# 2Retr0/GodotOceanWaves

Hardware: AMD Instinct MI355X
Metric: displacement+normal maps/sec, 1024^2 x 4 cascades; achieved HBM GB/s vs peak (higher is better)
Workload: dtype f32; 1 GPU; 1024^2 x 4 cascades per GPU, steady-state tick (modulate + 2-D IFFT + unpack/foam), delta=1/50 s, SURVEY 8d cascade table; map_size=1024, cascades_per_gpu=4, parallelism=cascade-sharded x1, gather=none

## Files before the change

godotoceanwaves_amd/_lib.py:

```python
import ctypes as C
import os

_HERE = os.path.dirname(os.path.abspath(__file__))
LIB_PATH = os.environ.get("OCEAN_WAVES_LIB") or os.path.join(_HERE, "libocean_waves.so")

OW_MAX_CASCADES = 8
OW_MAX_DEVICES = 8
OW_GROUP_FLAG_FORCE_PEER_PATH = 0x10000
OW_FLAG_DEBUG_F32 = 1
OW_FLAG_KERNELS_STANDARD = 2
OW_FLAG_KERNELS_LAYER_PARALLEL = 4
OW_FLAG_KERNELS_COMPACT = 8
OW_FLAG_NO_TICK_GROUPS = 16
OW_FLAG_RUN_AS_CALLS = 32
OW_FLAG_RUN_AS_REFERENCE_SCHEDULE = 64
OW_FLAG_GROUP_P1_LP, OW_FLAG_GROUP_P1_COMPACT, OW_FLAG_GROUP_P2_PLAIN, OW_FLAG_GROUP_P2_PIPE = 0x100, 0x200, 0x400, 0x800
OW_FLAG_ALWAYS_REGENERATE_SPECTRUM = 0x1000
OW_FLAG_LAZY_SCRATCH = 0x2000
OW_FLAG_SINGLE_STREAM = 0x4000
OW_FLAG_BODIES_FUSED, OW_FLAG_BODIES_SPLIT = 0x8000, 0x20000
OW_BODIES_MAX_SUBSTEPS = 64
OW_QUERY_DISTANCE_FALLOFF = 1
OW_BUOYANCY_WARM_START = 1
OW_BUOYANCY_WATER_VELOCITY = 2
# ... 140 lines not shown
SIGNATURES = {
    "ow_create": (C.c_int, [_P(ow_config), _P(C.c_void_p)]),
    "ow_destroy": (None, [C.c_void_p]),
    "ow_cascade_params_default": (None, [_P(ow_cascade_params)]),
    "ow_update": (C.c_int, [C.c_void_p, C.c_double, _P(ow_cascade_params), C.c_int32]),
    "ow_set_cascade_params": (C.c_int, [C.c_void_p, C.c_int32, _P(ow_cascade_params)]),
    "ow_get_cascade_params": (C.c_int, [C.c_void_p, C.c_int32, _P(ow_cascade_params)]),
    "ow_debug_inject_fault": (C.c_int, [C.c_void_p, C.c_uint32]),
    "ow_get_push_constants": (C.c_int, [C.c_void_p, C.c_int32, _P(ow_push_constants)]),
    "ow_process": (C.c_int, [C.c_void_p]),
    "ow_update_all": (C.c_int, [C.c_void_p, C.c_double, _P(ow_cascade_params), C.c_int32]),
    "ow_run": (C.c_int, [C.c_void_p, C.c_double, _P(ow_cascade_params), C.c_int32, C.c_int32]),
    "ow_lookahead_stats": (C.c_int, [C.c_void_p, _P(C.c_uint64), _P(C.c_uint64)]),
    "ow_spectrum_stats": (C.c_int, [C.c_void_p, _P(C.c_uint64), _P(C.c_uint64)]),
    "ow_chain_stats": (C.c_int, [C.c_void_p, _P(C.c_uint64)]),
    "ow_cascades_remaining": (C.c_int32, [C.c_void_p]),
    "ow_last_kernel_family": (C.c_int32, [C.c_void_p]),
    "ow_last_batch_cascades": (C.c_int32, [C.c_void_p]),
    "ow_tick_group_depth": (C.c_int32, [C.c_void_p]),
    "ow_sync": (C.c_int, [C.c_void_p]),
    "ow_get_device_ptrs": (C.c_int, [C.c_void_p, _P(C.c_void_p), _P(C.c_void_p), _P(C.c_size_t)]),
    "ow_get_maps": (C.c_int, [C.c_void_p, C.c_int32, C.c_void_p, C.c_void_p]),
    "ow_set_normal_map": (C.c_int, [C.c_void_p, C.c_int32, C.c_void_p]),
    "ow_readback_begin": (C.c_int, [C.c_void_p, C.c_uint32]),
    "ow_readback_wait": (C.c_int, [C.c_void_p, C.c_int32, _P(C.c_void_p), _P(C.c_void_p)]),
    "ow_sample_surface": (C.c_int, [C.c_void_p, C.c_void_p, C.c_int32, C.c_void_p, C.c_int32, C.c_void_p]),
    "ow_query_surface": (C.c_int, [C.c_void_p, C.c_void_p, C.c_int32, C.c_void_p, C.c_int32, _P(ow_query_options), C.c_void_p]),
    "ow_query_surface_async": (C.c_int, [C.c_void_p, C.c_void_p, C.c_int32, C.c_void_p, C.c_int32, _P(ow_query_options), C.c_void_p]),
    "ow_buoyancy": (C.c_int, [C.c_void_p, C.c_void_p, C.c_int32, C.c_void_p, C.c_int32, C.c_void_p, C.c_int32, _P(ow_buoyancy_options),
                              C.c_void_p, C.c_void_p]),
# ... 83 lines not shown
```

godotoceanwaves_amd/csrc/ow_device.h:

```cpp
#pragma once

#include <stdint.h>
#include <math.h>

#if defined(__HIPCC__)
#define OW_DEV __device__ __forceinline__
#define OW_HD __host__ __device__ __forceinline__
#define OW_DEVICE_BUILD 1
#define OW_SCHED_FENCE() __builtin_amdgcn_sched_barrier(0)
#else
#define OW_DEV inline
#define OW_HD inline
#define OW_DEVICE_BUILD 0
#define OW_SCHED_FENCE() ((void)0)
#endif

namespace ow {

#if OW_DEVICE_BUILD
typedef float cplx __attribute__((ext_vector_type(2)));
#else
struct alignas(8) cplx {
    float x, y;
};
// ... 467 lines not shown
#else
    return (uint32_t)f2h(lo) | ((uint32_t)f2h(hi) << 16);
#endif
}

struct CascadeFrame {
    float tile_x, tile_y;
    float time;
    float whitecap;
    float foam_grow_rate;
    float foam_decay;
    int32_t cascade;
    int32_t fault;
};
constexpr uint32_t kStatusRowSyncTimeout = 1u;
constexpr unsigned long long kRowSyncTimeoutTicks = 2000000ull;
constexpr int plan_lp_rows(int N) { return 128 / plan_T(N) > 0 ? 128 / plan_T(N) : 1; }
constexpr int plan_lp_threads(int N) { return plan_lp_rows(N) * kLayers * plan_T(N); }
constexpr int plan_lp_lds_cplx(int N) { return plan_region_cplx(N) * plan_lp_rows(N) * kLayers + plan_tw_total(N); }
constexpr int plan_lp_handoff_cplx(int N) { return plan_lp_threads(N) / 2; }

template <int N>
struct TickPlan {
    static constexpr int Q = plan_lp_threads(N) / plan_wg_threads(N);
    static constexpr int GPS = N / kWgRows;
    static_assert(Q >= 1 && plan_lp_threads(N) % plan_wg_threads(N) == 0 && (GPS / 2) % Q == 0, "block shapes of the two passes must nest");
    static constexpr int full(int slots) { return slots * GPS / Q; }
    static constexpr int upper(int slots) { return slots * (GPS / 2) / Q; }
    static constexpr int row0(int slots) { return (slots * 3 + Q - 1) / Q; }
    static constexpr int items_1(int slots) { return 2 * full(slots) + upper(slots) + row0(slots); }
// ... 51 lines not shown
struct PairArgs {
    PairFrame c[8];
    float time1[8];
    int32_t tbase2, tbase1;
    int32_t n2, n1;
    int32_t first2, first1;
    int32_t fault, pad;
};
OW_HD CascadeFrame pair_frame(const PairArgs &g, int launch_slot) {
    const PairFrame &f = g.c[launch_slot];
    CascadeFrame cf;
    cf.tile_x = f.tile_x, cf.tile_y = f.tile_y, cf.time = g.time1[launch_slot], cf.whitecap = f.whitecap;
    cf.foam_grow_rate = f.foam_grow_rate, cf.foam_decay = f.foam_decay, cf.cascade = f.cascade, cf.fault = g.fault;
    return cf;
}
constexpr int32_t kFaultRowSync = 1;
constexpr int kMaxCascades = 8;
struct FrameArgs {
    CascadeFrame c[kMaxCascades];
};

#if OW_DEVICE_BUILD
typedef uint32_t u32x4_t __attribute__((ext_vector_type(4)));
typedef uint32_t u32x2_t __attribute__((ext_vector_type(2)));
struct GBuf {
    __amdgpu_buffer_rsrc_t r;
};
OW_DEV GBuf make_gbuf(const void *base, uint32_t bytes) {
    return GBuf{__builtin_amdgcn_make_buffer_rsrc(const_cast<void *>(base), 0, (int)bytes, 0x00020000)};
}
// ... 332 lines not shown

    static OW_DEV uint32_t t_voff(int t, int xp) {
        return (T >= 16 ? t_unit(N, 0, xp, t) : t_unit(N, 0, xp, 0) + (uint32_t)t) * 8u;
    }
    static constexpr uint32_t t_soff(int layer, int j) {
        return (t_unit(N, layer, 0, 0) + (T >= 16 ? t_unit(N, 0, 0, T * j) : t_unit(N, 0, 0, 16 * (j / 2)) + 8u * (j % 2))) * 8u;
    }
    static constexpr int rot(int j) { return (j + 8) & 15; }
    template <int AUX>
    static OW_DEV void load_layer(cplx *d, int t, int xp, int layer, GBuf T_c) {
        const uint32_t voff = t_voff(t, xp);
#pragma unroll
        for (int j = 0; j < P; ++j) d[j] = gload8<AUX>(T_c, voff, t_soff(layer, rot(j)));
    }
    OW_HD static constexpr uint32_t foam_index(int xp, int yp) { return (uint32_t)xp * N + (uint32_t)(yp % T) * 16u + (uint32_t)(yp / T); }
    static OW_DEV void load_foam(uint32_t *pk, int t, int xp, GBuf foam_c) {
        const uint32_t voff = foam_index(xp, t) * 2u;
        const f32x4 a = gload16(foam_c, voff, 0u), b = gload16(foam_c, voff, 16u);
        const float v[8] = {a.x, a.y, a.z, a.w, b.x, b.y, b.z, b.w};
#pragma unroll
        for (int i = 0; i < 8; ++i) pk[i] = __builtin_bit_cast(uint32_t, v[i]);
    }
    static OW_DEV void store_foam(const uint32_t *pk, int t, int xp, GBuf foam_c) {
        const uint32_t voff = foam_index(xp, t) * 2u;
        float v[8];
#pragma unroll
        for (int i = 0; i < 8; ++i) v[i] = __builtin_bit_cast(float, pk[i]);
        gstore16(foam_c, voff, 0u, f32x4{v[0], v[1], v[2], v[3]});
        gstore16(foam_c, voff, 16u, f32x4{v[4], v[5], v[6], v[7]});
    }

    static OW_DEV void f32_put(GBuf f32_c, uint32_t tex, int o, int ch, float v) {
#if OW_DEVICE_BUILD
        __builtin_amdgcn_raw_buffer_store_b32(__builtin_bit_cast(uint32_t, v), f32_c.r, (int)(tex * 32u + (uint32_t)ch * 4u), (int)((uint32_t)(T * o) * 32u), 0);
#else
        __builtin_memcpy(f32_c.p + tex * 32u + (uint32_t)ch * 4u + (uint32_t)(T * o) * 32u, &v, 4);
#endif
    }

    template <bool F32>
    static OW_DEV void after_layer3(const cplx *l3, const cplx *l2, uint32_t *foam_pk, uint32_t *gy_foam,
                                    uint32_t tex, const CascadeFrame &cf, GBuf f32_c) {
#pragma unroll
        for (int o = 0; o < P; ++o) {
// ... 331 lines not shown
```

godotoceanwaves_amd/csrc/ow_frame.hip:

```cpp
#include <hip/hip_ext.h>

#include "ow_frame_kernels.h"

namespace ow {

template <class K, class... A>
static void launch(K kernel, dim3 grid, dim3 block, hipStream_t s, const LaunchTiming &lt, A... args) {
    if (lt.start) hipExtLaunchKernelGGL(kernel, grid, block, 0, s, lt.start, lt.stop, 0, args...);
    else hipLaunchKernelGGL(kernel, grid, block, 0, s, args...);
}

constexpr int kAutoLargeFamily = 3;

bool supported_map_size(int n) { return n == 128 || n == 256 || n == 512 || n == 1024 || n == 2048; }

template <int N>
static int family(int slots, int mode) {
    constexpr bool has_compact = plan_T(N) >= 16, has_lp_compact = plan_T(N) >= 16;
    if (mode == 1 || mode == 2) return mode;
    if (mode == 3) return has_compact ? 3 : 1;
    if (mode == 4) return has_lp_compact ? 4 : 2;
    const long waves = (long)slots * N * plan_T(N) / 64;
    if (has_lp_compact && waves >= 64 && waves <= 1536) return 4;
    if (waves <= 1024) return 2;
// ... 81 lines not shown
    g.n2 = g.slots2 * per2;
    g.n1 = g.slots1 * per1;
    if (g.n2 + g.n1 < 1) return hipErrorInvalidValue;
    PairArgs pa;
    for (int i = 0; i < kMaxCascades; ++i) {
        const CascadeFrame &cf = args.c[i];
        pa.c[i] = PairFrame{cf.tile_x, cf.tile_y, cf.whitecap, cf.foam_grow_rate, cf.foam_decay, cf.cascade};
        pa.time1[i] = g.time1[0][i];
    }
    pa.tbase2 = g.tbase2[0], pa.tbase1 = g.tbase1[0], pa.n2 = g.n2, pa.n1 = g.n1, pa.first2 = g.first2, pa.first1 = g.first1;
    pa.fault = args.c[0].fault, pa.pad = 0;
    if constexpr (plan_split(N)) launch(k_tick_pair_c_split<N, F32>, dim3(g.n2 + g.n1), dim3(PairSplitGeo<N>::kThreads), s, lt, buf, pa, (Stamp *)nullptr);
    else launch(k_tick_pair_c<N, F32>, dim3(g.n2 + g.n1), dim3(plan_wg_threads(N)), s, lt, buf, pa);
    return hipGetLastError();
}
template <int N, bool F32>
static hipError_t launch_group_n(const FrameArgs &args, TickGroupArgs g, const DeviceBuffers &buf, hipStream_t s, const LaunchTiming &lt, hipStream_t side) {
    using TP = TickPlan<N>;
    if (g.pair_compact) return launch_pair_n<N, F32>(args, g, buf, s, lt, side);
    if (plan_lp_rows(N) < 2) g.p2_pipe = 0;
    if (g.slots < 1 || g.first1 < 0 || g.step1 < 0 || g.first1 + (g.d1 > 0 ? g.d1 - 1 : 0) * g.step1 + g.slots > kMaxCascades) return hipErrorInvalidValue;
    g.n2 = g.d2 > 0 ? (g.p2_pipe ? TP::items_2_pipe(g.slots) : TP::items_2(g.slots)) : 0;
    g.n1 = g.p1_compact ? TP::items_1_compact(g.slots) : TP::items_1(g.slots);
    const int blocks = g.n2 + g.d1 * g.n1;
    if (blocks < 1) return hipErrorInvalidValue;
    if (g.p2_pipe) launch(k_tick_group_c_lp<N, F32, false, true>, dim3(blocks), dim3(plan_lp_threads(N)), s, lt, buf, args, g, (Stamp *)nullptr);
    else launch(k_tick_group_c_lp<N, F32>, dim3(blocks), dim3(plan_lp_threads(N)), s, lt, buf, args, g, (Stamp *)nullptr);
    return hipGetLastError();
}
bool tick_groups_supported(int n) { return n == 256 || n == 512 || n == 1024; }
// ... 54 lines not shown
```

godotoceanwaves_amd/csrc/ow_frame_kernels.h:

```cpp
#pragma once
#include <type_traits>

#include "ow_kernels.h"

#ifndef OW_P1_WAVES
#define OW_P1_WAVES 4
#endif
namespace ow {

struct Stamp {
    unsigned long long t[16];
    unsigned xcc, pad;
    unsigned long long rt0, rt1;
};
struct DebugArgs {
    Stamp *stamps;
    int never_true;
};

__device__ __forceinline__ void wave_sync() {
    __builtin_amdgcn_fence(__ATOMIC_RELEASE, "wavefront");
    __builtin_amdgcn_wave_barrier();
    __builtin_amdgcn_fence(__ATOMIC_ACQUIRE, "wavefront");
}
// ... 443 lines not shown
    const GBuf rrow_c = make_gbuf(buf.rrow + (size_t)tslot * N * 4, (uint32_t)N * 32u);

    cplx h[P];
    const float dkx = (2.0f * kPi) / cf.tile_x, dky = (2.0f * kPi) / cf.tile_y;
    const float ky = (float)(y - N / 2) * dky;
    float ik[P];
    {
        cplx a[P], b[P];
        float om[P];
        Pass1<N>::template load_raw<AUX_H>(a, b, om, t, y, h0_c, om_c);
        issued();
        Pass1<N>::modulate(h, a, b, om, time);
    }
    stamp(1, h[0].x);
    Pass1<N>::wave_numbers(ik, t, ky, dkx);
    if (t == 0) gstore8(pcol_c, Pass2<N>::pcol_index(y) * 8u, 0u, Pass1<N>::column_term(h, ik, t, dkx));

    if (__builtin_amdgcn_readfirstlane(y) == 0) {
#pragma unroll
        for (int Q = 1; Q <= 3; ++Q) {
            cplx d[P];
            OW_SCHED_FENCE();
            {
                const float kyo = opaque(ky), dkxo = opaque(dkx);
                const int to = opaque(t);
#pragma unroll
                for (int j = 0; j < P; ++j) opaque_inplace(h[j]);
                if (Q == 1) Pass1<N>::template row0_input<1>(d, h, ik, to, kyo, dkxo);
                if (Q == 2) Pass1<N>::template row0_input<2>(d, h, ik, to, kyo, dkxo);
                if (Q == 3) Pass1<N>::template row0_input<3>(d, h, ik, to, kyo, dkxo);
            }
            OW_SCHED_FENCE();
            row_ifft<N, false>(d, t, lds_row, tw_lds, rs);
            rs.sync();
            if (y == 0) {
#pragma unroll
                for (int o = 0; o < P; ++o) gstore8(rrow_c, (uint32_t)(t + Tn * o) * 32u, (uint32_t)Q * 8u, d[OutMap<N>::slot_of(o)]);
            }
        }
    }

    const bool lower = row0 < N / 2;
#pragma unroll
    for (int L = 0; L < LC; ++L) {
        if (L == 1 && lower) continue;
        cplx d[P];
        OW_SCHED_FENCE();
        {
            const float kyo = opaque(ky), dkxo = opaque(dkx);
            const int to = opaque(t);
#pragma unroll
            for (int j = 0; j < P; ++j) opaque_inplace(h[j]);
// ... 69 lines not shown
                                            RS &rs, Issued issued, uint32_t (&foam_pk)[kP / 2], int foam_io = 3) {
    constexpr int Tn = plan_T(N), P = kP;
    constexpr bool TWH = p2c_half_table(N);
    const int rw = (Tn >= 64) ? __builtin_amdgcn_readfirstlane(tau / Tn) : tau / Tn, t = tau % Tn;
    const uint32_t plane = (uint32_t)N * N;
    cplx *lds_row = rows_lds + rw * plan_region_cplx(N);
    const int xp = row0 + rw;
    const GBuf T_c = make_gbuf(buf.T + (size_t)tslot * plane * kLayers, t_cascade_bytes(N));
    const GBuf pcol_c = make_gbuf(buf.pcol + (size_t)tslot * N, (uint32_t)N * 8u);
    const GBuf rrow_c = make_gbuf(buf.rrow + (size_t)tslot * N * 4, (uint32_t)N * 32u);
    const GBuf disp_c = make_gbuf(buf.disp + (size_t)cf.cascade * plane, plane * 8u);
    const GBuf norm_c = make_gbuf(buf.norm + (size_t)cf.cascade * plane, plane * 8u);
    const GBuf foam_c = make_gbuf(buf.foam + (size_t)cf.cascade * plane, plane * 2u);
    const GBuf f32_c = make_gbuf(F32 ? buf.f32 + (size_t)cf.cascade * plane * 8 : nullptr, F32 ? plane * 32u : 0u);
    const float dky = (2.0f * kPi) / cf.tile_y;
    auto side_row = [&](int q) { return gload8(rrow_c, (uint32_t)xp * 32u, (uint32_t)q * 8u); };

    uint32_t hz_pk[P / 2];
    float c2[P];
    {
        cplx f2[P];
        OW_SCHED_FENCE();
        Pass2<N>::template load_c1<AUX_T>(f2, t, xp, dky, T_c);
        const cplx r2 = side_row(2);
        issued();
        Pass2<N>::put_row0(f2, t, r2);
        row_ifft<N, false, TWH>(f2, opaque(t), lds_row, tw_lds, rs);
        OW_SCHED_FENCE();
        Pass2<N>::template after_f2<F32>(f2, hz_pk, c2, (uint32_t)(xp * N + opaque(t)), f32_c);
    }
    cplx c0[P];
// ... 2 lines not shown
        OW_SCHED_FENCE();
        const int tq = opaque(t);
        Pass2<N>::template load_layer<AUX_T>(c0, tq, xp, 0, T_c);
#pragma unroll
        for (int j = 0; j < P; ++j) f0[j] = c0[j];
        row_ifft<N, false, TWH>(f0, opaque(t), lds_row, tw_lds, rs);
        OW_SCHED_FENCE();
        const int tr = opaque(t);
        Pass2<N>::template after_f0<F32, AUX_O>(f0, hz_pk, tr, xp, (uint32_t)(xp * N + tr), disp_c, f32_c);
    }
    float dhx_dx[P];
    uint32_t gx_pk[P / 2];
    {
        OW_SCHED_FENCE();
        const int tq = opaque(t);
        Pass2<N>::derive_dx(c0, tq, xp, dky, pcol_c);
        Pass2<N>::put_row0(c0, tq, side_row(1));
        row_ifft<N, false, TWH>(c0, opaque(t), lds_row, tw_lds, rs);
        OW_SCHED_FENCE();
        Pass2<N>::template after_f1<F32>(c0, dhx_dx, gx_pk, (uint32_t)(xp * N + opaque(t)), f32_c);
    }
    {
        cplx f3[P];
        OW_SCHED_FENCE();
        const int tq = opaque(t);
        Pass2<N>::template load_layer<AUX_T>(f3, tq, xp, 2, T_c);
        Pass2<N>::put_row0(f3, tq, side_row(3));
        if (foam_io & 1) Pass2<N>::load_foam(foam_pk, tq, xp, foam_c);
        row_ifft<N, false, TWH>(f3, opaque(t), lds_row, tw_lds, rs);
        OW_SCHED_FENCE();
        const int tr = opaque(t);
        Pass2<N>::template after_f3<F32, AUX_O>(f3, dhx_dx, c2, gx_pk, foam_pk, (uint32_t)(xp * N + tr), cf, norm_c, f32_c);
        if (foam_io & 2) Pass2<N>::store_foam(foam_pk, tr, xp, foam_c);
    }
}

template <int N, bool F32, int AUX_T = kAuxDefault, int AUX_O = kAuxDefault>
__global__ __launch_bounds__(plan_wg_threads(N), 4) void k_pass2c(DeviceBuffers buf, FrameArgs args) {
    constexpr int Tn = plan_T(N);
    static_assert(Tn >= 16, "Pass2::load_c1 needs N/16 to be a multiple of the 16-row line");
    constexpr int TW = p2c_table_total(N), ROWS_CPLX = plan_region_cplx(N) * kWgRows;
    __shared__ __attribute__((aligned(16))) cplx lds[TW + ROWS_CPLX + plan_sync_flag_cplx(N, kWgRows)];
    cplx *tw_lds = lds;
    cplx *rows_lds = lds + TW;
    const int tau = threadIdx.x;
    int *sync_flags = reinterpret_cast<int *>(lds + TW + ROWS_CPLX);
    RowSync<N> rs;
    rs.attach(sync_flags, tau / Tn, (tau / 64) & 1);
// ... 709 lines not shown
    } else {
        p1_index_to_rows<N>(index, slot, row0);
    }
    const int launch_slot = (first ? g.first1 : g.first2) + slot;
    const CascadeFrame cf = pair_frame(g, launch_slot);
    fetch_arguments(buf, cf);
    if (!first) {
        uint32_t foam_pk[kP / 2];
        pass2c_item<N, F32, kAuxDefault, kAuxNT>(buf, cf, g.tbase2 + slot, row0, (int)threadIdx.x, tw_lds, rows_lds, rs, [&] { tw_commit<N>(twp, tw_lds); }, foam_pk);
    } else {
        pass1c_item<N, kAuxDefault, kAuxDefault>(buf, cf, g.time1[launch_slot], g.tbase1 + slot, row0, (int)threadIdx.x, tw_lds, rows_lds, rs,
                                                 [&] { tw_commit<N>(twp, tw_lds); }, [](int, float) {});
    }
}

}
```

godotoceanwaves_amd/csrc/ow_kernels.h:

```cpp
#pragma once
#include <hip/hip_runtime.h>

#include "ow_device.h"
#include "ow_buoyancy.h"
#include "ow_raycast.h"
#include "ow_render.h"
#include "ow_rigid.h"
#include "ow_surface.h"
#include "ow_velocity.h"
#include "ow_velocity_kernels.h"

namespace ow {

struct DeviceBuffers {
    cplx *h0;
    float *omega;
    cplx *T;
    u16x4 *disp;
    u16x4 *norm;
    uint16_t *foam;
    float *f32;
    const cplx *tw;
    cplx *pcol;
    cplx *rrow;
// ... 37 lines not shown

bool supported_map_size(int n);
int kernel_family(int n, int slots, int mode);
hipError_t launch_spectrum(int n, int cascade, const SpectrumPC &pc, const DeviceBuffers &buf, hipStream_t s);
hipError_t launch_pass1(int n, int slots, int mode, const FrameArgs &args, const DeviceBuffers &buf, hipStream_t s,
                        const LaunchTiming &lt = LaunchTiming{});
hipError_t launch_pass2(int n, int slots, int mode, const FrameArgs &args, const DeviceBuffers &buf, hipStream_t s,
                        const LaunchTiming &lt = LaunchTiming{});

bool tick_groups_supported(int n);
bool tick_pairs_supported(int n);
int tick_group_pipe_blocks(int n, int slots);
hipError_t launch_tick_group(int n, const FrameArgs &args, const TickGroupArgs &g, const DeviceBuffers &buf, hipStream_t s,
                             const LaunchTiming &lt = LaunchTiming{}, hipStream_t side = nullptr);
bool tick_pair_splits(int n, const TickGroupArgs &g);

}
```

godotoceanwaves_amd/csrc/ow_runtime.hip:

```cpp
#include <hip/hip_runtime.h>
#include <unistd.h>

#include <algorithm>
#include <cmath>
#include <cstdarg>
#include <cstddef>
#include <cstdio>
#include <cstring>
#include <new>
#include <string>
#include <vector>

#include "ow_internal.h"
#include "ow_kernels.h"
#include "ow_tables.h"

namespace {
thread_local std::string g_last_error;
}

namespace ow {
ow_status fail(ow_status st, const char *fmt, ...) {
    char buf[512];
    va_list ap;
// ... 20 lines not shown
    uint64_t substeps = 0, fused_launches = 0, split_calls = 0;
};

struct ow_context {
    int n = 0, cascades = 0, layers = 0, device = 0;
    float depth = 20.0f;
    int kernel_mode = 0;
    int last_family = 0;
    int bodies_mode = 0;
    hipStream_t stream = nullptr;
    bool own_stream = false, own_disp = false, own_norm = false;
    hipStream_t side_stream = nullptr;
    hipEvent_t side_fork_ev = nullptr, side_join_ev = nullptr;
    bool side_active = false;
    uint64_t split_launches = 0;
    ow::DeviceBuffers buf{};
    ow::cplx *tw_dev = nullptr, *tw_split_dev = nullptr, *tw_half_dev = nullptr;
    ow_cascade_params pass_parameters[OW_MAX_CASCADES] = {};
    int pass_count = 0;
    int pass_num_cascades_remaining = 0;
    uint32_t *status_host = nullptr;
    uint32_t inject_fault = 0;
    uint32_t maps_faulted = 0, enqueued_since_sync = 0;
    uint32_t readback_faulted = 0;
    ow_push_constants pc_words[OW_MAX_CASCADES] = {};
    bool pc_valid[OW_MAX_CASCADES] = {};
    bool spectrum_resident[OW_MAX_CASCADES] = {};
    bool always_regenerate = false;
    uint64_t spectra_generated = 0, spectra_skipped = 0;
    struct Lookahead {
// ... 64 lines not shown
    ow::RaycastHit *ray_out = nullptr;
    int ray_capacity = 0;
    uint32_t *ray_bound = nullptr;
    uint32_t *render_rgba = nullptr;
    ow::RenderPixel *render_pixels = nullptr;
    size_t render_rgba_capacity = 0, render_pixels_capacity = 0;
    ow::u16x4 *vel = nullptr;
    ow::cplx *vel_scratch = nullptr, *vel_tw = nullptr;
    int vel_slots = 0;
    uint32_t velocity_stale = 0, spectrum_ahead = 0;
    uint64_t vel_computed = 0, vel_skipped = 0;
    std::vector<ow_bodies *> body_sets;
    uint64_t host_syncs = 0;
};

static hipStream_t main_stream(ow_context *c) {
    if (c->side_active && hipEventRecord(c->side_join_ev, c->side_stream) == hipSuccess && hipStreamWaitEvent(c->stream, c->side_join_ev, 0) == hipSuccess)
        c->side_active = false;
    return c->stream;
}
static bool side_fork(ow_context *c) {
    if (c->side_active) return true;
    if (hipEventRecord(c->side_fork_ev, c->stream) != hipSuccess || hipStreamWaitEvent(c->side_stream, c->side_fork_ev, 0) != hipSuccess) {
        (void)hipGetLastError();
        return false;
    }
    c->side_active = true;
    return true;
}
static bool may_split(const ow_context *c) {
    const int min_run = c->n >= 1024 ? 8 : 16;
    return c->side_stream && (c->own_stream || (c->inside_run && !c->run_as_calls && !c->run_as_reference && c->run_frames >= min_run));
}
static hipError_t launch_group(ow_context *c, const ow::FrameArgs &args, const ow::TickGroupArgs &ga, const ow::LaunchTiming &lt = ow::LaunchTiming{}) {
    if (may_split(c) && !lt.start && ow::tick_pair_splits(c->n, ga) && side_fork(c)) {
        ++c->split_launches;
        return ow::launch_tick_group(c->n, args, ga, c->buf, c->stream, lt, c->side_stream);
    }
    return ow::launch_tick_group(c->n, args, ga, c->buf, main_stream(c), lt);
}
static void join_for_caller(ow_context *c) {
    if (!c->own_stream) (void)main_stream(c);
}

namespace {

size_t plane(const ow_context *c) { return (size_t)c->n * c->n; }

constexpr size_t kSinglePairTexels = 6u << 20, kBatchTexels = 4u << 20;
// ... 133 lines not shown
}

ow_status consume_status(ow_context *c) {
    if (!c->status_host || *c->status_host == 0u) {
        return OW_OK;
    }
    const uint32_t bits = *c->status_host;
    *c->status_host = 0u;
    c->maps_faulted |= c->enqueued_since_sync;
    c->enqueued_since_sync = 0;
    c->la.queued = 0;
    c->ra.armed = false;
    for (int i = 0; i < OW_MAX_CASCADES; ++i)
        if (c->copy_pending[i]) c->readback_faulted |= 1u << i;
    return fail(OW_ERR_HIP, "device-side failure reported by a frame kernel (status 0x%x%s): the maps of the batches enqueued since "
                            "the last synchronisation are invalid", bits, (bits & ow::kStatusRowSyncTimeout) ? ": wave-pair rendezvous timed out" : "");
}
ow_status refuse_faulted(const ow_context *c, uint32_t layer_mask) {
    if (c->maps_faulted & layer_mask)
        return fail(OW_ERR_HIP, "layer mask 0x%x holds maps of a batch that reported a device-side failure (already returned by an earlier call); "
                                "they stay invalid until a later batch has recomputed those layers (faulted: 0x%x)", layer_mask, c->maps_faulted);
    return OW_OK;
}
ow_status sync_stream(ow_context *c, uint32_t layer_mask) {
    ++c->host_syncs;
    OW_HIP(hipStreamSynchronize(main_stream(c)));
    if (ow_status st = consume_status(c); st != OW_OK) return st;
    c->enqueued_since_sync = 0;
    return refuse_faulted(c, layer_mask);
}

// ... 522 lines not shown
        ow_destroy(c);
        return st;
    };
    if (cfg->stream) {
        c->stream = (hipStream_t)cfg->stream;
    } else {
        if (hipStreamCreateWithFlags(&c->stream, hipStreamNonBlocking) != hipSuccess)
            return bail(fail(OW_ERR_HIP, "hipStreamCreate failed"));
        c->own_stream = true;
    }
    if (!(cfg->flags & OW_FLAG_SINGLE_STREAM) && ((c->n == 1024 && c->cascades >= 4) || (c->n == 512 && c->cascades >= 8))) {
        if (hipStreamCreateWithFlags(&c->side_stream, hipStreamNonBlocking) != hipSuccess || hipEventCreateWithFlags(&c->side_fork_ev, hipEventDisableTiming) != hipSuccess ||
            hipEventCreateWithFlags(&c->side_join_ev, hipEventDisableTiming) != hipSuccess)
            return bail(fail(OW_ERR_HIP, "second stream / events: creation failed"));
    }
    const size_t pl = plane(c), L = (size_t)c->layers;
#define OW_ALLOC(ptr, bytes)                                                                              \
    if (hipMalloc((void **)&(ptr), (bytes)) != hipSuccess)                                                \
        return bail(fail(OW_ERR_NOMEM, "hipMalloc of %zu bytes failed for " #ptr, (size_t)(bytes)));
    OW_ALLOC(c->buf.h0, L * pl * sizeof(ow::cplx));
    OW_ALLOC(c->buf.omega, L * pl * sizeof(float));
    c->no_merge = (cfg->flags & OW_FLAG_NO_TICK_GROUPS) != 0;
    c->run_as_calls = (cfg->flags & OW_FLAG_RUN_AS_CALLS) != 0;
    c->run_as_reference = (cfg->flags & OW_FLAG_RUN_AS_REFERENCE_SCHEDULE) != 0;
    c->always_regenerate = (cfg->flags & OW_FLAG_ALWAYS_REGENERATE_SPECTRUM) != 0;
    plan_tick_groups(c, cfg->flags);
    const bool lazy_scratch = (cfg->flags & OW_FLAG_LAZY_SCRATCH) != 0;
    if (ensure_scratch(c, lazy_scratch ? base_scratch_slots(c) : std::max(base_scratch_slots(c), lookahead_scratch_slots(c))) != OW_OK) return bail(OW_ERR_NOMEM);
    if (cfg->displacement_map) {
        c->buf.disp = (ow::u16x4 *)cfg->displacement_map;
    } else {
        OW_ALLOC(c->buf.disp, exportable_bytes(L * pl * sizeof(ow::u16x4)));
        c->own_disp = true;
    }
    if (cfg->normal_map) {
        c->buf.norm = (ow::u16x4 *)cfg->normal_map;
    } else {
        OW_ALLOC(c->buf.norm, exportable_bytes(L * pl * sizeof(ow::u16x4)));
        c->own_norm = true;
    }
    OW_ALLOC(c->buf.foam, L * pl * sizeof(uint16_t));
    if (cfg->flags & OW_FLAG_DEBUG_F32) { OW_ALLOC(c->buf.f32, L * pl * 8 * sizeof(float)); }
    if (hipHostMalloc((void **)&c->status_host, 64, hipHostMallocMapped) != hipSuccess)
        return bail(fail(OW_ERR_NOMEM, "hipHostMalloc failed for the device status word"));
    *c->status_host = 0u;
    if (hipHostGetDevicePointer((void **)&c->buf.status, c->status_host, 0) != hipSuccess)
        return bail(fail(OW_ERR_HIP, "hipHostGetDevicePointer failed for the device status word"));
    std::vector<ow::cplx> tw;
    ow::make_twiddles(c->n, tw);
    OW_ALLOC(c->tw_dev, tw.size() * sizeof(ow::cplx));
    std::vector<ow::cplx> tw_split;
    if (ow::make_split_twiddles(c->n, tw_split)) { OW_ALLOC(c->tw_split_dev, tw_split.size() * sizeof(ow::cplx)); }
    std::vector<ow::cplx> tw_half;
    if (ow::make_half_twiddles(c->n, tw_half)) { OW_ALLOC(c->tw_half_dev, tw_half.size() * sizeof(ow::cplx)); }
#undef OW_ALLOC
    c->buf.tw = c->tw_dev;
// ... 22 lines not shown
    (void)hipGetDevice(&caller_dev);
    (void)hipSetDevice(c->device);
    if (c->side_stream) (void)hipStreamSynchronize(c->side_stream);
    if (c->stream) (void)hipStreamSynchronize(c->stream);
    for (ow_bodies *set : c->body_sets) {
        (void)hipFree(set->block);
        set->block = nullptr;
        set->ctx = nullptr;
    }
    (void)hipFree(c->buf.h0);
    (void)hipFree(c->buf.omega);
    (void)hipFree(c->buf.T);
    if (c->own_disp) (void)hipFree(c->buf.disp);
    if (c->own_norm) (void)hipFree(c->buf.norm);
    (void)hipFree(c->buf.foam);
    (void)hipFree(c->buf.f32);
    (void)hipFree(c->buf.pcol);
    (void)hipFree(c->buf.rrow);
    (void)hipFree(c->tw_dev);
    (void)hipFree(c->tw_split_dev);
    (void)hipFree(c->tw_half_dev);
    if (c->status_host) (void)hipHostFree(c->status_host);
    if (c->copy_stream) (void)hipStreamSynchronize(c->copy_stream);
    (void)hipFree(c->snap_dev);
    if (c->snap_host) (void)hipHostFree(c->snap_host);
    for (auto &e : c->snap_ready)
        if (e) (void)hipEventDestroy(e);
    for (auto &e : c->copy_done)
        if (e) (void)hipEventDestroy(e);
    if (c->copy_stream) (void)hipStreamDestroy(c->copy_stream);
// ... 113 lines not shown
    return OW_OK;
}

ow_status ow_update_all(ow_context *c, double delta, ow_cascade_params *params, int32_t count) {
    ow_status st = update_impl(c, delta, params, count, false);
    if (st != OW_OK) return st;
    int idx[OW_MAX_CASCADES];
    for (int i = 0; i < count; ++i) idx[i] = count - 1 - i;
    if (!lookahead_tick(c, delta, count, &st)) st = enqueue(c, c->pass_parameters, idx, count);
    if (st != OW_OK) return st;
    c->pass_num_cascades_remaining = 0;
    if (!c->inside_run) join_for_caller(c);
    return OW_OK;
}

ow_status ow_chain_stats(const ow_context *c, uint64_t *split_launches) {
    if (!c) return fail(OW_ERR_INVALID, "null context");
    if (split_launches) *split_launches = c->split_launches;
    return OW_OK;
}

ow_status ow_lookahead_stats(const ow_context *c, uint64_t *hits, uint64_t *speculated) {
    if (!c) return fail(OW_ERR_INVALID, "null context");
    if (hits) *hits = c->la.hits;
    if (speculated) *speculated = c->la.speculated;
    return OW_OK;
}

ow_status ow_spectrum_stats(const ow_context *c, uint64_t *generated, uint64_t *skipped) {
    if (!c) return fail(OW_ERR_INVALID, "null context");
// ... 261 lines not shown
ow_status run_impl(ow_context *c, double delta, ow_cascade_params *params, int32_t count, int32_t frames) {
    auto delta_of = [&](int tick) { return c->run_delta_period > 0 && ((tick / c->run_delta_period) & 1) ? delta * 1.25 : delta; };
    if (c->run_as_reference) {
        for (int f = 0; f < frames; ++f) {
            if (ow_status st = ow_update(c, delta_of(f), params, count); st != OW_OK) return st;
            for (int k = 0; k < count; ++k)
                if (ow_status st = ow_process(c); st != OW_OK) return st;
        }
        return OW_OK;
    }
    int f = 0;
    const bool may_merge = !c->run_as_calls && !c->no_merge && std::isfinite(delta) && count >= 1 && count <= c->cascades;
    if (frames >= 3 && may_merge && c->timing == 0 && lookahead_mode(c, count) == 1) {
        const uint64_t before = c->la.hits + c->la.speculated;
        ow_status st = OW_OK;
        for (; f < frames && st == OW_OK; ++f) {
            c->la.certain = frames - f - 1;
            st = ow_update_all(c, delta, params, count);
        }
        c->la.certain = 0;
        if (st != OW_OK) return st;
        if (c->la.hits + c->la.speculated != before) {
            c->last_family = 6;
            c->last_group_depth = 1;
        }
        return OW_OK;
    }
    const bool speculate = may_merge && c->ra.run_streak >= 1 && c->timing == 0 && !c->inject_fault;
    if (may_merge && frames >= 1 && c->ra.armed) {
        const int depth = run_resume_usable(c, delta, params, count, frames);
        if (depth != 0) {
            OW_HIP(hipSetDevice(c->device));
            for (int i = 0; i < count; ++i) (void)settle_spectrum(c, i, params[i], false);
            note_cadence(c, delta);
            return depth > 0 ? run_tick_groups(c, delta, params, count, frames, depth, true, speculate) : run_tick_pairs(c, delta, params, count, frames, true, speculate);
// ... 1249 lines not shown
```

godotoceanwaves_amd/wave_generator.py:

```python
import ctypes as C
import math

import numpy as np

from . import _lib
from ._lib import (OW_FLAG_ALWAYS_REGENERATE_SPECTRUM, OW_FLAG_LAZY_SCRATCH, OW_FLAG_SINGLE_STREAM, OW_FLAG_DEBUG_F32, OW_FLAG_GROUP_P1_COMPACT, OW_FLAG_GROUP_P1_LP, OW_FLAG_GROUP_P2_PIPE, OW_FLAG_GROUP_P2_PLAIN, OW_FLAG_KERNELS_COMPACT,
                   OW_FLAG_KERNELS_LAYER_PARALLEL, OW_FLAG_KERNELS_STANDARD, OW_FLAG_NO_TICK_GROUPS, OW_FLAG_RUN_AS_CALLS, OW_FLAG_RUN_AS_REFERENCE_SCHEDULE,
                   ow_cascade_params, ow_config)

G = 9.81
DEPTH = 20.0


def _dirty(name, clamp=None):
    attr = "_" + name

    def getter(self):
        return getattr(self, attr)

    def setter(self, value):
        setattr(self, attr, clamp(value) if clamp else value)
        self.should_generate_spectrum = True

    return property(getter, setter)
# ... 590 lines not shown
        return int(self._lib.ow_last_batch_cascades(self.context))

    def tick_group_depth(self):
        return int(self._lib.ow_tick_group_depth(self.context))

    def lookahead_stats(self):
        h, sp = C.c_uint64(), C.c_uint64()
        _lib.check(self._lib.ow_lookahead_stats(self.context, C.byref(h), C.byref(sp)))
        return h.value, sp.value

    def chain_stats(self):
        n = C.c_uint64()
        _lib.check(self._lib.ow_chain_stats(self.context, C.byref(n)))
        return n.value

    def spectrum_stats(self):
        g, sk = C.c_uint64(), C.c_uint64()
        _lib.check(self._lib.ow_spectrum_stats(self.context, C.byref(g), C.byref(sk)))
        return g.value, sk.value

    def timing(self, enable):
        _lib.check(self._lib.ow_timing_enable(self.context, 2 if enable == 2 else (1 if enable else 0)))

    def probe_kernel_times(self, reps=50):
        a, b, n = C.c_float(), C.c_float(), C.c_int32()
        _lib.check(self._lib.ow_probe_kernel_times(self.context, reps, C.byref(a), C.byref(b), C.byref(n)))
        return a.value, b.value, n.value

    def timing_read_launches(self, reset=True):
        a, n = C.c_float(), C.c_int32()
# ... 8 lines not shown
```

include/ocean_waves.h:

```cpp
#ifndef OCEAN_WAVES_H
#define OCEAN_WAVES_H

#include <stddef.h>
#include <stdint.h>

#ifdef __cplusplus
extern "C" {
#endif

#define OW_MAX_CASCADES 8
#define OW_MAX_DEVICES 8
#define OW_ABI_VERSION 4

typedef enum ow_status {
    OW_OK = 0,
    OW_ERR_INVALID = 1,
    OW_ERR_NO_DEVICE = 2,
    OW_ERR_HIP = 3,
    OW_ERR_NOMEM = 4,
    OW_ERR_STATE = 5
} ow_status;

typedef struct ow_cascade_params {
    float tile_length[2];
// ... 54 lines not shown
void ow_cascade_params_default(ow_cascade_params *p);


ow_status ow_update(ow_context *ctx, double delta, ow_cascade_params *params, int32_t count);

ow_status ow_set_cascade_params(ow_context *ctx, int32_t index, const ow_cascade_params *params);
ow_status ow_get_cascade_params(const ow_context *ctx, int32_t index, ow_cascade_params *out);

ow_status ow_process(ow_context *ctx);

ow_status ow_update_all(ow_context *ctx, double delta, ow_cascade_params *params, int32_t count);
ow_status ow_lookahead_stats(const ow_context *ctx, uint64_t *hits, uint64_t *speculated);

ow_status ow_spectrum_stats(const ow_context *ctx, uint64_t *generated, uint64_t *skipped);
ow_status ow_chain_stats(const ow_context *ctx, uint64_t *split_launches);

ow_status ow_run(ow_context *ctx, double delta, ow_cascade_params *params, int32_t count, int32_t frames);

int32_t ow_cascades_remaining(const ow_context *ctx);

ow_status ow_sync(ow_context *ctx);


ow_status ow_get_device_ptrs(ow_context *ctx, void **displacement_map, void **normal_map, size_t *layer_stride_bytes);

ow_status ow_get_maps(ow_context *ctx, int32_t cascade, void *displacement_rgba16f, void *normal_rgba16f);

ow_status ow_set_normal_map(ow_context *ctx, int32_t cascade, const void *normal_rgba16f);


// ... 371 lines not shown
```

Before: 82920 maps/s.

## Batch consecutive tick pairs into one persistent dependency-counted run kernel

Adds a tick-run kernel that collects up to 32 consecutive compact pair ticks on the host and launches them as a single grid. Work items are handed out through atomic ticket counters, optionally one queue per XCD, and each item spins on per-cascade completion counters until the pass it depends on is done. This replaces per-tick kernel launches and stream ordering with in-kernel dataflow synchronisation, so passes from different ticks can overlap. Cross-block data now goes through agent-scope cache-policy loads and stores instead of fences. The risks are polling overhead and a timeout path that aborts the run and sets a fault status if a wait takes too long.

```diff
diff --git a/godotoceanwaves_amd/_lib.py b/godotoceanwaves_amd/_lib.py
--- a/godotoceanwaves_amd/_lib.py
+++ b/godotoceanwaves_amd/_lib.py
@@ -178,6 +178,7 @@
     "ow_lookahead_stats": (C.c_int, [C.c_void_p, _P(C.c_uint64), _P(C.c_uint64)]),
     "ow_spectrum_stats": (C.c_int, [C.c_void_p, _P(C.c_uint64), _P(C.c_uint64)]),
     "ow_chain_stats": (C.c_int, [C.c_void_p, _P(C.c_uint64)]),
+    "ow_run_kernel_stats": (C.c_int, [C.c_void_p, _P(C.c_uint64), _P(C.c_uint64)]),
     "ow_cascades_remaining": (C.c_int32, [C.c_void_p]),
     "ow_last_kernel_family": (C.c_int32, [C.c_void_p]),
     "ow_last_batch_cascades": (C.c_int32, [C.c_void_p]),
diff --git a/godotoceanwaves_amd/csrc/ow_device.h b/godotoceanwaves_amd/csrc/ow_device.h
--- a/godotoceanwaves_amd/csrc/ow_device.h
+++ b/godotoceanwaves_amd/csrc/ow_device.h
@@ -505,6 +505,7 @@
     int32_t fault;
 };
 constexpr uint32_t kStatusRowSyncTimeout = 1u;
+constexpr uint32_t kStatusRunWaitTimeout = 2u;
 constexpr unsigned long long kRowSyncTimeoutTicks = 2000000ull;
 constexpr int plan_lp_rows(int N) { return 128 / plan_T(N) > 0 ? 128 / plan_T(N) : 1; }
 constexpr int plan_lp_threads(int N) { return plan_lp_rows(N) * kLayers * plan_T(N); }
@@ -586,6 +587,23 @@
     cf.foam_grow_rate = f.foam_grow_rate, cf.foam_decay = f.foam_decay, cf.cascade = f.cascade, cf.fault = g.fault;
     return cf;
 }
+constexpr int kMaxRunTicks = 32;
+constexpr int kRunDone2 = 0;
+constexpr int kRunDone1 = 8;
+constexpr int kRunFault = 24;
+constexpr int kRunCounterWords = 64;
+constexpr int kRunTickets = 64;
+constexpr int kRunFinished = 72;
+constexpr int kRunSyncWords = 128;
+constexpr uint32_t kRunWaitPolls = 1u << 17;
+struct RunArgs {
+    PairFrame c[8];
+    float time1[kMaxRunTicks][8];
+    int32_t tbase2[kMaxRunTicks], tbase1[kMaxRunTicks];
+    int32_t slots, ticks;
+    int32_t queues, pad;
+    uint32_t *sync;
+};
 constexpr int32_t kFaultRowSync = 1;
 constexpr int kMaxCascades = 8;
 struct FrameArgs {
@@ -948,20 +966,22 @@
         for (int j = 0; j < P; ++j) d[j] = gload8<AUX>(T_c, voff, t_soff(layer, rot(j)));
     }
     OW_HD static constexpr uint32_t foam_index(int xp, int yp) { return (uint32_t)xp * N + (uint32_t)(yp % T) * 16u + (uint32_t)(yp / T); }
+    template <int AUX = 0>
     static OW_DEV void load_foam(uint32_t *pk, int t, int xp, GBuf foam_c) {
         const uint32_t voff = foam_index(xp, t) * 2u;
-        const f32x4 a = gload16(foam_c, voff, 0u), b = gload16(foam_c, voff, 16u);
+        const f32x4 a = gload16<AUX>(foam_c, voff, 0u), b = gload16<AUX>(foam_c, voff, 16u);
         const float v[8] = {a.x, a.y, a.z, a.w, b.x, b.y, b.z, b.w};
 #pragma unroll
         for (int i = 0; i < 8; ++i) pk[i] = __builtin_bit_cast(uint32_t, v[i]);
     }
+    template <int AUX = 0>
     static OW_DEV void store_foam(const uint32_t *pk, int t, int xp, GBuf foam_c) {
         const uint32_t voff = foam_index(xp, t) * 2u;
         float v[8];
 #pragma unroll
         for (int i = 0; i < 8; ++i) v[i] = __builtin_bit_cast(float, pk[i]);
-        gstore16(foam_c, voff, 0u, f32x4{v[0], v[1], v[2], v[3]});
-        gstore16(foam_c, voff, 16u, f32x4{v[4], v[5], v[6], v[7]});
+        gstore16<AUX>(foam_c, voff, 0u, f32x4{v[0], v[1], v[2], v[3]});
+        gstore16<AUX>(foam_c, voff, 16u, f32x4{v[4], v[5], v[6], v[7]});
     }
 
     static OW_DEV void f32_put(GBuf f32_c, uint32_t tex, int o, int ch, float v) {
diff --git a/godotoceanwaves_amd/csrc/ow_frame.hip b/godotoceanwaves_amd/csrc/ow_frame.hip
--- a/godotoceanwaves_amd/csrc/ow_frame.hip
+++ b/godotoceanwaves_amd/csrc/ow_frame.hip
@@ -119,6 +119,23 @@
     else launch(k_tick_pair_c<N, F32>, dim3(g.n2 + g.n1), dim3(plan_wg_threads(N)), s, lt, buf, pa);
     return hipGetLastError();
 }
+template <int N>
+static hipError_t launch_run_n(const RunArgs &g, const DeviceBuffers &buf, hipStream_t s) {
+    const int blocks = g.ticks * 2 * g.slots * (N / kWgRows);
+    if (buf.f32) launch(k_tick_run_c<N, true>, dim3(blocks), dim3(plan_wg_threads(N)), s, LaunchTiming{}, buf, g);
+    else launch(k_tick_run_c<N, false>, dim3(blocks), dim3(plan_wg_threads(N)), s, LaunchTiming{}, buf, g);
+    return hipGetLastError();
+}
+bool tick_run_supported(int n) { return n == 256 || n == 512 || n == 1024; }
+hipError_t launch_tick_run(int n, const RunArgs &g, const DeviceBuffers &buf, hipStream_t s) {
+    if (g.slots < 1 || g.slots > kMaxCascades || g.ticks < 1 || g.ticks > kMaxRunTicks || (g.queues != 1 && g.queues != 8) || !g.sync) return hipErrorInvalidValue;
+    switch (n) {
+        case 256: return launch_run_n<256>(g, buf, s);
+        case 512: return launch_run_n<512>(g, buf, s);
+        case 1024: return launch_run_n<1024>(g, buf, s);
+    }
+    return hipErrorInvalidValue;
+}
 template <int N, bool F32>
 static hipError_t launch_group_n(const FrameArgs &args, TickGroupArgs g, const DeviceBuffers &buf, hipStream_t s, const LaunchTiming &lt, hipStream_t side) {
     using TP = TickPlan<N>;
diff --git a/godotoceanwaves_amd/csrc/ow_frame_kernels.h b/godotoceanwaves_amd/csrc/ow_frame_kernels.h
--- a/godotoceanwaves_amd/csrc/ow_frame_kernels.h
+++ b/godotoceanwaves_amd/csrc/ow_frame_kernels.h
@@ -481,7 +481,7 @@
     }
     stamp(1, h[0].x);
     Pass1<N>::wave_numbers(ik, t, ky, dkx);
-    if (t == 0) gstore8(pcol_c, Pass2<N>::pcol_index(y) * 8u, 0u, Pass1<N>::column_term(h, ik, t, dkx));
+    if (t == 0) gstore8<AUX_T>(pcol_c, Pass2<N>::pcol_index(y) * 8u, 0u, Pass1<N>::column_term(h, ik, t, dkx));
 
     if (__builtin_amdgcn_readfirstlane(y) == 0) {
 #pragma unroll
@@ -502,7 +502,7 @@
             rs.sync();
             if (y == 0) {
 #pragma unroll
-                for (int o = 0; o < P; ++o) gstore8(rrow_c, (uint32_t)(t + Tn * o) * 32u, (uint32_t)Q * 8u, d[OutMap<N>::slot_of(o)]);
+                for (int o = 0; o < P; ++o) gstore8<AUX_T>(rrow_c, (uint32_t)(t + Tn * o) * 32u, (uint32_t)Q * 8u, d[OutMap<N>::slot_of(o)]);
             }
         }
     }
@@ -602,7 +602,7 @@
     const GBuf foam_c = make_gbuf(buf.foam + (size_t)cf.cascade * plane, plane * 2u);
     const GBuf f32_c = make_gbuf(F32 ? buf.f32 + (size_t)cf.cascade * plane * 8 : nullptr, F32 ? plane * 32u : 0u);
     const float dky = (2.0f * kPi) / cf.tile_y;
-    auto side_row = [&](int q) { return gload8(rrow_c, (uint32_t)xp * 32u, (uint32_t)q * 8u); };
+    auto side_row = [&](int q) { return gload8<AUX_T>(rrow_c, (uint32_t)xp * 32u, (uint32_t)q * 8u); };
 
     uint32_t hz_pk[P / 2];
     float c2[P];
@@ -635,7 +635,7 @@
     {
         OW_SCHED_FENCE();
         const int tq = opaque(t);
-        Pass2<N>::derive_dx(c0, tq, xp, dky, pcol_c);
+        Pass2<N>::template derive_dx<AUX_T>(c0, tq, xp, dky, pcol_c);
         Pass2<N>::put_row0(c0, tq, side_row(1));
         row_ifft<N, false, TWH>(c0, opaque(t), lds_row, tw_lds, rs);
         OW_SCHED_FENCE();
@@ -647,12 +647,12 @@
         const int tq = opaque(t);
         Pass2<N>::template load_layer<AUX_T>(f3, tq, xp, 2, T_c);
         Pass2<N>::put_row0(f3, tq, side_row(3));
-        if (foam_io & 1) Pass2<N>::load_foam(foam_pk, tq, xp, foam_c);
+        if (foam_io & 1) Pass2<N>::template load_foam<AUX_T>(foam_pk, tq, xp, foam_c);
         row_ifft<N, false, TWH>(f3, opaque(t), lds_row, tw_lds, rs);
         OW_SCHED_FENCE();
         const int tr = opaque(t);
         Pass2<N>::template after_f3<F32, AUX_O>(f3, dhx_dx, c2, gx_pk, foam_pk, (uint32_t)(xp * N + tr), cf, norm_c, f32_c);
-        if (foam_io & 2) Pass2<N>::store_foam(foam_pk, tr, xp, foam_c);
+        if (foam_io & 2) Pass2<N>::template store_foam<AUX_T>(foam_pk, tr, xp, foam_c);
     }
 }
 
@@ -1392,4 +1392,112 @@
     }
 }
 
-}
+#ifndef OW_RUN_FENCES
+#define OW_RUN_FENCES 0
+#endif
+template <int N, bool F32>
+__global__ __launch_bounds__(plan_wg_threads(N), 4) void k_tick_run_c(DeviceBuffers buf, RunArgs g) {
+    static_assert(!plan_row_spans_waves(N), "N <= 1024");
+    static_assert(kRunDone1 + 2 * 8 <= kRunFault && kRunFault < 64 && kRunCounterWords == 64, "one wave loads every counter at once");
+    constexpr int PER = N / kWgRows;
+    constexpr int AUX_X = OW_RUN_FENCES ? kAuxDefault : kAuxAgent;
+    __shared__ __attribute__((aligned(16))) cplx lds[plan_wg_lds_cplx(N)];
+    __shared__ int drawn[2];
+    cplx *tw_lds = lds;
+    cplx *rows_lds = lds + plan_tw_total(N);
+    RowSync<N> rs;
+    TwPrefetch<N> twp;
+    tw_fetch<N>(twp, buf.tw);
+    const int per_pair = 2 * g.slots * PER, total = g.ticks * per_pair, per_queue = total / g.queues;
+    auto counter = [&](int w) { return __hip_atomic_load(g.sync + w, __ATOMIC_RELAXED, __HIP_MEMORY_SCOPE_AGENT); };
+    auto decode = [&](int item, int &j, bool &first, int &slot, int &row0) {
+        j = item / per_pair;
+        int index = item - j * per_pair;
+        first = (index >> 3) & 1;
+        index = ((index >> 4) << 3) + (index & 7);
+        if (!first) {
+            slot = index / PER;
+            row0 = (index % PER) * kWgRows;
+        } else {
+            p1_index_to_rows<N>(index, slot, row0);
+        }
+    };
+    if (threadIdx.x < 64) {
+        const int lane = threadIdx.x;
+        uint32_t cv = counter(lane);
+        int item = -1;
+        const int q0 = g.queues > 1 ? (int)(xcc_id() % (unsigned)g.queues) : 0;
+        for (int i = 0; i < g.queues && item < 0; ++i) {
+            const int q = (q0 + i) % g.queues;
+            uint32_t tk = 0;
+            if (lane == 0) tk = __hip_atomic_fetch_add(g.sync + kRunTickets + q, 1u, __ATOMIC_RELAXED, __HIP_MEMORY_SCOPE_AGENT);
+            tk = __builtin_amdgcn_readfirstlane(tk);
+            if (tk < (uint32_t)per_queue) item = (int)tk * g.queues + q;
+        }
+        bool skip = __shfl(cv, kRunFault) != 0u || item < 0, gave_up = item < 0;
+        if (!skip) {
+            int j, slot, row0;
+            bool first;
+            decode(item, j, first, slot, row0);
+            if (j > 0) {
+                const int w2 = kRunDone2 + slot, w1 = kRunDone1 + 2 * slot + ((j - 1) & 1);
+                const uint32_t need2 = (uint32_t)j * PER, need1 = first ? 0u : (uint32_t)((j - 1) / 2 + 1) * PER;
+                uint32_t c2 = __shfl(cv, w2), c1 = __shfl(cv, w1);
+                for (uint32_t polls = 0; c2 < need2 || c1 < need1;) {
+                    if (++polls > kRunWaitPolls) {
+                        skip = gave_up = true;
+                        break;
+                    }
+                    __builtin_amdgcn_s_sleep(8);
+                    c2 = counter(w2), c1 = counter(w1);
+                    if (counter(kRunFault) != 0u) {
+                        skip = true;
+                        break;
+                    }
+                }
+            }
+        }
+        if (gave_up && lane == 0) {
+            __hip_atomic_store(g.sync + kRunFault, 1u, __ATOMIC_RELAXED, __HIP_MEMORY_SCOPE_AGENT);
+            __hip_atomic_store(buf.status, kStatusRunWaitTimeout, __ATOMIC_RELAXED, __HIP_MEMORY_SCOPE_SYSTEM);
+            __threadfence_system();
+        }
+        if (lane == 0) drawn[0] = item, drawn[1] = skip;
+    }
+    __syncthreads();
+    const int item = __builtin_amdgcn_readfirstlane(drawn[0]);
+    const bool skip = __builtin_amdgcn_readfirstlane(drawn[1]) != 0;
+    int j = 0, slot = 0, row0 = 0;
+    bool first = false;
+    if (item >= 0) decode(item, j, first, slot, row0);
+    if (!skip) {
+        if (OW_RUN_FENCES && j > 0) __builtin_amdgcn_fence(__ATOMIC_ACQUIRE, "agent");
+        const PairFrame &f = g.c[slot];
+        CascadeFrame cf;
+        cf.tile_x = f.tile_x, cf.tile_y = f.tile_y, cf.time = g.time1[j][slot], cf.whitecap = f.whitecap;
+        cf.foam_grow_rate = f.foam_grow_rate, cf.foam_decay = f.foam_decay, cf.cascade = f.cascade, cf.fault = 0;
+        fetch_arguments(buf, cf);
+        if (!first) {
+            uint32_t foam_pk[kP / 2];
+            pass2c_item<N, F32, AUX_X, kAuxNT>(buf, cf, g.tbase2[j] + slot, row0, (int)threadIdx.x, tw_lds, rows_lds, rs, [&] { tw_commit<N>(twp, tw_lds); }, foam_pk);
+        } else {
+            pass1c_item<N, AUX_X, kAuxDefault>(buf, cf, cf.time, g.tbase1[j] + slot, row0, (int)threadIdx.x, tw_lds, rows_lds, rs, [&] { tw_commit<N>(twp, tw_lds); },
+                                               [](int, float) {});
+        }
+        if (OW_RUN_FENCES) __builtin_amdgcn_fence(__ATOMIC_RELEASE, "agent");
+    }
+    asm volatile("s_waitcnt vmcnt(0)" ::: "memory");
+    __syncthreads();
+    if (threadIdx.x == 0) {
+        if (item >= 0) {
+            const int w = first ? kRunDone1 + 2 * slot + (j & 1) : kRunDone2 + slot;
+            const uint32_t before = __hip_atomic_fetch_add(g.sync + w, 1u, __ATOMIC_RELAXED, __HIP_MEMORY_SCOPE_AGENT);
+            asm volatile("" ::"v"(before));
+        }
+        if (__hip_atomic_fetch_add(g.sync + kRunFinished, 1u, __ATOMIC_RELAXED, __HIP_MEMORY_SCOPE_AGENT) == (uint32_t)total - 1u) {
+            for (int w = 0; w < kRunSyncWords; ++w) __hip_atomic_store(g.sync + w, 0u, __ATOMIC_RELAXED, __HIP_MEMORY_SCOPE_AGENT);
+        }
+    }
+}
+
+}
diff --git a/godotoceanwaves_amd/csrc/ow_kernels.h b/godotoceanwaves_amd/csrc/ow_kernels.h
--- a/godotoceanwaves_amd/csrc/ow_kernels.h
+++ b/godotoceanwaves_amd/csrc/ow_kernels.h
@@ -75,5 +75,7 @@
 hipError_t launch_tick_group(int n, const FrameArgs &args, const TickGroupArgs &g, const DeviceBuffers &buf, hipStream_t s,
                              const LaunchTiming &lt = LaunchTiming{}, hipStream_t side = nullptr);
 bool tick_pair_splits(int n, const TickGroupArgs &g);
+bool tick_run_supported(int n);
+hipError_t launch_tick_run(int n, const RunArgs &g, const DeviceBuffers &buf, hipStream_t s);
 
 }
diff --git a/godotoceanwaves_amd/csrc/ow_runtime.hip b/godotoceanwaves_amd/csrc/ow_runtime.hip
--- a/godotoceanwaves_amd/csrc/ow_runtime.hip
+++ b/godotoceanwaves_amd/csrc/ow_runtime.hip
@@ -58,6 +58,13 @@
     hipEvent_t side_fork_ev = nullptr, side_join_ev = nullptr;
     bool side_active = false;
     uint64_t split_launches = 0;
+    bool single_stream = false;
+    bool run_collect = false;
+    ow::RunArgs run_pending{};
+    uint32_t *run_sync = nullptr;
+    int run_queues = 1;
+    hipError_t run_error = hipSuccess;
+    uint64_t run_launches = 0, run_ticks = 0;
     ow::DeviceBuffers buf{};
     ow::cplx *tw_dev = nullptr, *tw_split_dev = nullptr, *tw_half_dev = nullptr;
     ow_cascade_params pass_parameters[OW_MAX_CASCADES] = {};
@@ -152,10 +159,50 @@
     uint64_t host_syncs = 0;
 };
 
-static hipStream_t main_stream(ow_context *c) {
+static hipStream_t joined_stream(ow_context *c) {
     if (c->side_active && hipEventRecord(c->side_join_ev, c->side_stream) == hipSuccess && hipStreamWaitEvent(c->stream, c->side_join_ev, 0) == hipSuccess)
         c->side_active = false;
     return c->stream;
+}
+static void flush_run(ow_context *c) {
+    if (c->run_pending.ticks == 0) return;
+    c->run_pending.sync = c->run_sync;
+    c->run_pending.queues = c->run_queues;
+    const hipError_t e = ow::launch_tick_run(c->n, c->run_pending, c->buf, joined_stream(c));
+    if (e == hipSuccess) {
+        ++c->run_launches;
+        c->run_ticks += (uint64_t)c->run_pending.ticks;
+    } else {
+        (void)hipGetLastError();
+        c->run_error = e;
+    }
+    c->run_pending.ticks = 0;
+}
+static hipStream_t main_stream(ow_context *c) {
+    flush_run(c);
+    return joined_stream(c);
+}
+static bool collect_for_run(ow_context *c, const ow::FrameArgs &args, const ow::TickGroupArgs &ga) {
+    if (!c->run_collect || c->la.certain < 1 || !ga.pair_compact || ga.d2 != 1 || ga.d1 != 1 || ga.slots2 < 1 || ga.slots1 != ga.slots2 || ga.first2 != 0 || ga.first1 != 0 || args.c[0].fault != 0)
+        return false;
+    ow::PairFrame frames[ow::kMaxCascades] = {};
+    for (int i = 0; i < ga.slots2; ++i) {
+        const ow::CascadeFrame &cf = args.c[i];
+        frames[i] = ow::PairFrame{cf.tile_x, cf.tile_y, cf.whitecap, cf.foam_grow_rate, cf.foam_decay, cf.cascade};
+    }
+    ow::RunArgs &g = c->run_pending;
+    if (g.ticks > 0 && (g.slots != ga.slots2 || std::memcmp(g.c, frames, sizeof(frames)) != 0)) flush_run(c);
+    if (g.ticks == 0) {
+        std::memset(&g, 0, sizeof(g));
+        std::memcpy(g.c, frames, sizeof(frames));
+        g.slots = ga.slots2;
+    }
+    const int j = g.ticks++;
+    for (int i = 0; i < ow::kMaxCascades; ++i) g.time1[j][i] = ga.time1[0][i];
+    g.tbase2[j] = ga.tbase2[0];
+    g.tbase1[j] = ga.tbase1[0];
+    if (g.ticks == ow::kMaxRunTicks) flush_run(c);
+    return true;
 }
 static bool side_fork(ow_context *c) {
     if (c->side_active) return true;
@@ -171,6 +218,8 @@
     return c->side_stream && (c->own_stream || (c->inside_run && !c->run_as_calls && !c->run_as_reference && c->run_frames >= min_run));
 }
 static hipError_t launch_group(ow_context *c, const ow::FrameArgs &args, const ow::TickGroupArgs &ga, const ow::LaunchTiming &lt = ow::LaunchTiming{}) {
+    if (!lt.start && collect_for_run(c, args, ga)) return hipSuccess;
+    flush_run(c);
     if (may_split(c) && !lt.start && ow::tick_pair_splits(c->n, ga) && side_fork(c)) {
         ++c->split_launches;
         return ow::launch_tick_group(c->n, args, ga, c->buf, c->stream, lt, c->side_stream);
@@ -334,7 +383,7 @@
     for (int i = 0; i < OW_MAX_CASCADES; ++i)
         if (c->copy_pending[i]) c->readback_faulted |= 1u << i;
     return fail(OW_ERR_HIP, "device-side failure reported by a frame kernel (status 0x%x%s): the maps of the batches enqueued since "
-                            "the last synchronisation are invalid", bits, (bits & ow::kStatusRowSyncTimeout) ? ": wave-pair rendezvous timed out" : "");
+                            "the last synchronisation are invalid", bits, (bits & ow::kStatusRowSyncTimeout) ? ": wave-pair rendezvous timed out" : (bits & ow::kStatusRunWaitTimeout) ? ": an item of the tick-run kernel gave up waiting" : "");
 }
 ow_status refuse_faulted(const ow_context *c, uint32_t layer_mask) {
     if (c->maps_faulted & layer_mask)
@@ -887,6 +936,7 @@
             hipEventCreateWithFlags(&c->side_join_ev, hipEventDisableTiming) != hipSuccess)
             return bail(fail(OW_ERR_HIP, "second stream / events: creation failed"));
     }
+    c->single_stream = (cfg->flags & OW_FLAG_SINGLE_STREAM) != 0;
     const size_t pl = plane(c), L = (size_t)c->layers;
 #define OW_ALLOC(ptr, bytes)                                                                              \
     if (hipMalloc((void **)&(ptr), (bytes)) != hipSuccess)                                                \
@@ -913,6 +963,14 @@
         c->own_norm = true;
     }
     OW_ALLOC(c->buf.foam, L * pl * sizeof(uint16_t));
+    if (ow::tick_run_supported(c->n)) {
+        int cus = 0;
+        if (hipDeviceGetAttribute(&cus, hipDeviceAttributeMultiprocessorCount, c->device) != hipSuccess) cus = 0;
+        c->run_queues = cus == 256 ? 8 : 1;
+        OW_ALLOC(c->run_sync, ow::kRunSyncWords * sizeof(uint32_t));
+        if (hipMemsetAsync(c->run_sync, 0, ow::kRunSyncWords * sizeof(uint32_t), main_stream(c)) != hipSuccess)
+            return bail(fail(OW_ERR_HIP, "clearing the run kernel's counters failed"));
+    }
     if (cfg->flags & OW_FLAG_DEBUG_F32) { OW_ALLOC(c->buf.f32, L * pl * 8 * sizeof(float)); }
     if (hipHostMalloc((void **)&c->status_host, 64, hipHostMallocMapped) != hipSuccess)
         return bail(fail(OW_ERR_NOMEM, "hipHostMalloc failed for the device status word"));
@@ -965,6 +1023,7 @@
     if (c->own_disp) (void)hipFree(c->buf.disp);
     if (c->own_norm) (void)hipFree(c->buf.norm);
     (void)hipFree(c->buf.foam);
+    (void)hipFree(c->run_sync);
     (void)hipFree(c->buf.f32);
     (void)hipFree(c->buf.pcol);
     (void)hipFree(c->buf.rrow);
@@ -1108,6 +1167,12 @@
     return OW_OK;
 }
 
+ow_status ow_run_kernel_stats(const ow_context *c, uint64_t *launches, uint64_t *ticks) {
+    if (!c) return fail(OW_ERR_INVALID, "null context");
+    if (launches) *launches = c->run_launches;
+    if (ticks) *ticks = c->run_ticks;
+    return OW_OK;
+}
 ow_status ow_chain_stats(const ow_context *c, uint64_t *split_launches) {
     if (!c) return fail(OW_ERR_INVALID, "null context");
     if (split_launches) *split_launches = c->split_launches;
@@ -1399,11 +1464,22 @@
     if (frames >= 3 && may_merge && c->timing == 0 && lookahead_mode(c, count) == 1) {
         const uint64_t before = c->la.hits + c->la.speculated;
         ow_status st = OW_OK;
+#ifndef OW_NO_TICK_RUN
+        c->run_collect = c->run_sync != nullptr && !c->single_stream;
+#endif
         for (; f < frames && st == OW_OK; ++f) {
             c->la.certain = frames - f - 1;
             st = ow_update_all(c, delta, params, count);
         }
         c->la.certain = 0;
+        c->run_collect = false;
+        flush_run(c);
+        if (c->run_error != hipSuccess) {
+            const hipError_t e = c->run_error;
+            c->run_error = hipSuccess;
+            c->la.queued = 0;
+            if (st == OW_OK) st = fail(OW_ERR_HIP, "tick-run launch failed: %s", hipGetErrorString(e));
+        }
         if (st != OW_OK) return st;
         if (c->la.hits + c->la.speculated != before) {
             c->last_family = 6;
diff --git a/godotoceanwaves_amd/wave_generator.py b/godotoceanwaves_amd/wave_generator.py
--- a/godotoceanwaves_amd/wave_generator.py
+++ b/godotoceanwaves_amd/wave_generator.py
@@ -628,6 +628,11 @@
         _lib.check(self._lib.ow_chain_stats(self.context, C.byref(n)))
         return n.value
 
+    def run_kernel_stats(self):
+        n, t = C.c_uint64(), C.c_uint64()
+        _lib.check(self._lib.ow_run_kernel_stats(self.context, C.byref(n), C.byref(t)))
+        return n.value, t.value
+
     def spectrum_stats(self):
         g, sk = C.c_uint64(), C.c_uint64()
         _lib.check(self._lib.ow_spectrum_stats(self.context, C.byref(g), C.byref(sk)))
diff --git a/include/ocean_waves.h b/include/ocean_waves.h
--- a/include/ocean_waves.h
+++ b/include/ocean_waves.h
@@ -92,6 +92,7 @@
 
 ow_status ow_spectrum_stats(const ow_context *ctx, uint64_t *generated, uint64_t *skipped);
 ow_status ow_chain_stats(const ow_context *ctx, uint64_t *split_launches);
+ow_status ow_run_kernel_stats(const ow_context *ctx, uint64_t *launches, uint64_t *ticks);
 
 ow_status ow_run(ow_context *ctx, double delta, ow_cascade_params *params, int32_t count, int32_t frames);
 
```

Result: slower. 49250 maps/s (-40.6%).
